# avabag01-ai/spectrogram-midi

Hardware: AMD Instinct MI355X
Metric: audio-seconds transcribed/sec (44.1 kHz, n_fft=2048) (higher is better)
Workload: dtype f64

## Files before the change

spectrogram-midi_amd/csrc/frame.hip:

```cpp
#include "kernels.h"
#include "fft8.h"
#include "frame_walk.h"
#include "pass_geometry.h"
#include "wave_ops.h"

#include <algorithm>
#include <cfloat>
#include <cmath>
#include <cstdlib>
#include <cstring>

namespace aegis {

constexpr int kFramesPerWg = 16;

constexpr size_t kFrameLdsFixed = (size_t)2048 * 16 + 2048 * 4 + 1040 * 4 + 128 * 4 + 16 * 4 + 256 * 4;

#if defined(AEGIS_ABLATE) && (AEGIS_ABLATE & 128)
__device__ long long g_frm_dbg[24];
#define FRM_TICK(k) { __builtin_amdgcn_s_waitcnt(0); const long long now__ = clock64(); facc[k] += now__ - flast; flast = now__; }
#else
#define FRM_TICK(k)
#endif
template <bool INJECT>
__global__ __launch_bounds__(256, 2) void frame_yin_kernel(PassParams p, DevTables tb, int frames_per_wg, int en_stride,
                                                           const double *__restrict__ inj) {
#if defined(AEGIS_ABLATE) && (AEGIS_ABLATE & 128)
    long long facc[12] = {0, 0, 0, 0, 0, 0, 0, 0, 0, 0, 0, 0}, flast = clock64();
#endif
    extern __shared__ __align__(16) unsigned char fsm[];
    double2 *z = reinterpret_cast<double2 *>(fsm);
    float *xs = reinterpret_cast<float *>(z + 2048);
    float *pw = xs + 2048;
    float *red = pw + 1040;
    float *blk = red + 128;
    float *part = blk + 16;
    float *en = part + 256;
    int64_t *frow = reinterpret_cast<int64_t *>(en + (size_t)frames_per_wg * en_stride);

    const int tid = threadIdx.x, lane = tid & 63, wid = tid >> 6;
    const int64_t n_sel = geo_n_sel(p);
    const int64_t fs0 = (int64_t)blockIdx.x * frames_per_wg;
    if (fs0 >= n_sel) return;
    const int nfr = (int)min((int64_t)frames_per_wg, n_sel - fs0);
    const bool want_pyin = (p.stages & 0x4u) != 0, want_mel = (p.stages & 0x3u) != 0;
    const bool want_rms = (p.stages & 0x8u) && p.out_rms != nullptr;
    const bool want_fft = (p.stages & 0x7u) != 0;
    const int mp = p.max_period;

    struct Geo { bool live; int c; int64_t base, n, start, f, o; };
    auto locate = [&](int i) {
        Geo g{false, 0, 0, 0, 0, 0, 0};
        g.live = i < nfr;
        if (g.live) {
            int64_t t;
            map_frame(p, fs0 + i, g.c, t, g.f);
            g.o = out_index(p, g.c, t);
            g.base = p.sample_off[g.c];
            g.n = p.sample_len[g.c];
            g.start = t * p.hop - 1024;
        }
        return g;
    };
    auto fetch = [&](const Geo &g, float (&v)[8]) {
#pragma unroll
        for (int r = 0; r < 8; ++r) {
            const int64_t idx = g.start + tid + r * 256;
            v[r] = (g.live && idx >= 0 && idx < g.n) ? p.pcm[g.base + idx] : 0.0f;
        }
    };
    auto locate_next = [&](const Geo &g, int i, int64_t sel_end) {
        if (i < nfr && g.live && fs0 + i < sel_end) {
            Geo n = g;
            n.start += p.hop; n.f += 1; n.o += 1;
            return n;
        }
        return locate(i);
    };
    Geo geo = locate(0);
    int64_t geo_sel_end = geo.live ? p.sel_off[geo.c + 1] : 0;
    float nx[8];
    fetch(geo, nx);
    Fft8Tw twr;

    const bool has_chunk = want_mel && tid < tb.mel_chunks;
    const int mel_bin = has_chunk ? tb.mel_chunk_bin[tid] : 0;
    int band_c0 = 0, band_c1 = 0;
    if (want_mel && (tid & 127) < p.n_mels) { band_c0 = tb.mel_band_chunk[tid & 127]; band_c1 = tb.mel_band_chunk[(tid & 127) + 1]; }
    float *pw1 = xs;
    float *part1 = xs + 1040;
    if (tid < 15) pw[1025 + tid] = 0.0f;

    if (want_pyin) {
        const Geo g0 = geo;
        Geo gl = g0;
        if (fs0 + nfr - 1 < geo_sel_end) { gl.start += (int64_t)(nfr - 1) * p.hop; } else gl = locate(nfr - 1);
        const int64_t span = (int64_t)(nfr - 1) * p.hop + 2048;
        const bool staged = g0.c == gl.c && p.hop == 512 && span + 4 * (span >> 9) <= 10240;
        float *stage = reinterpret_cast<float *>(z);
        if (staged) {
            const float *__restrict__ x0 = p.pcm + g0.base;
            const int n4 = (int)(span >> 2);
            float4 sv[10];
#pragma unroll
            for (int u = 0; u < 10; ++u) {
                const int q = tid + 256 * u;
                const int64_t idx = g0.start + 4 * (int64_t)q;
                float4 v = make_float4(0.0f, 0.0f, 0.0f, 0.0f);
                if (q < n4) {
                    if (idx >= 0 && idx + 3 < g0.n) {
                        typedef float f4u __attribute__((ext_vector_type(4), aligned(4)));
                        const f4u t = *reinterpret_cast<const f4u *>(x0 + idx);
                        v = make_float4(t.x, t.y, t.z, t.w);
                    } else {
                        if (idx >= 0 && idx < g0.n) v.x = x0[idx];
                        if (idx + 1 >= 0 && idx + 1 < g0.n) v.y = x0[idx + 1];
                        if (idx + 2 >= 0 && idx + 2 < g0.n) v.z = x0[idx + 2];
                        if (idx + 3 >= 0 && idx + 3 < g0.n) v.w = x0[idx + 3];
                    }
                }
                sv[u] = v;
            }
#pragma unroll
            for (int u = 0; u < 10; ++u) {
                const int q = tid + 256 * u;
                if (q < n4) {
                    const int i = 4 * q;
                    *reinterpret_cast<float4 *>(stage + i + 4 * (i >> 9)) =
                        make_float4(sv[u].x * sv[u].x, sv[u].y * sv[u].y, sv[u].z * sv[u].z, sv[u].w * sv[u].w);
                }
            }
            __syncthreads();
        }
        if (wid == 0) __builtin_amdgcn_s_setprio(3);
        if (wid == 0 && lane < nfr) {
            float *row = en + lane * en_stride;
            if (staged) {
                const float *srow = stage + lane * (512 + 4);
                energy_walk<true>([&](int j, float4 &a, float4 &b) {
                    const float *q = srow + j + 4 * (j >> 9);
                    a = *reinterpret_cast<const float4 *>(q);
                    b = *reinterpret_cast<const float4 *>(q + 4);
                }, row, mp);
            } else {
                const Geo g = locate(lane);
                const float *__restrict__ x = p.pcm + g.base;
                energy_walk_plain([&](int j) {
                    const int64_t q = g.start + j;
                    return (q >= 0 && q < g.n) ? x[q] : 0.0f;
                }, row, mp);
            }
        }
        if (wid == 0) __builtin_amdgcn_s_setprio(0);
        if (staged) __syncthreads();
    }
    if (want_fft) fft8_load_twiddles(twr, tb.twiddle, tid);
    FRM_TICK(0)
    __builtin_amdgcn_s_waitcnt(kWaitVmcnt0);

    for (int pr = 0; pr < nfr; pr += 2) {
        double2 P[2][4], Pn[2];
        int64_t fidx[2] = {0, 0};
        int64_t fout[2] = {0, 0};
        bool flive[2] = {false, false};
        int fclip[2] = {0, 0};
#pragma unroll
        for (int h = 0; h < 2; ++h) {
#pragma unroll
            for (int r = 0; r < 4; ++r) P[h][r] = make_double2(0.0, 0.0);
            Pn[h] = make_double2(0.0, 0.0);
            if (pr + h >= nfr) continue;
            const bool live = geo.live;
            const int c = geo.c;
            const int64_t f = geo.f, fo = geo.o;
            fidx[h] = f; flive[h] = live; fclip[h] = c;
            if constexpr (INJECT) fout[h] = fo;
            if (tid == 0) frow[pr + h] = live ? f : -1;
#pragma unroll
            for (int r = 0; r < 8; ++r) xs[tid + r * 256] = nx[r];
            {
                const int cprev = geo.c;
                geo = locate_next(geo, pr + h + 1, geo_sel_end);
                if (geo.live && geo.c != cprev) geo_sel_end = p.sel_off[geo.c + 1];
            }
            fetch(geo, nx);
            __syncthreads();
            FRM_TICK(1)

            if (want_rms && tid < 128) {
                const int bb = tid >> 3, a = tid & 7;
                const float *xb = xs + bb * 128 + a;
                float r = xb[0] * xb[0];
#pragma unroll
                for (int i = 1; i < 16; ++i) { const float v = xb[8 * i]; r = r + v * v; }
                red[tid] = r;
            }
            if (!want_fft) {
                __syncthreads();
                if (want_rms && tid < 16) {
                    const float *r = red + tid * 8;
                    blk[tid] = ((r[0] + r[1]) + (r[2] + r[3])) + ((r[4] + r[5]) + (r[6] + r[7]));
                }
                __syncthreads();
            } else {
                double2 v[8];
#pragma unroll
                for (int q = 0; q < 8; ++q) {
                    const int i = tid + 256 * q;
                    v[q] = make_double2((double)xs[i], i < 1024 ? (double)xs[1024 - i] : 0.0);
                }
                fft8_pass1_write(z, tid, v);
                __syncthreads();
                if (want_rms && tid < 16) {
                    const float *r = red + tid * 8;
                    blk[tid] = ((r[0] + r[1]) + (r[2] + r[3])) + ((r[4] + r[5]) + (r[6] + r[7]));
                }
                fft8_read8(z, tid, v);
                __syncthreads();
                fft8_pass_write<8>(z, tid, v, twr.p2);
                __syncthreads();
                fft8_read8(z, tid, v);
                __syncthreads();
                fft8_pass_write<64>(z, tid, v, twr.p3);
                __syncthreads();
                fft8_pass4(z, tid, twr);
                __syncthreads();
            }
            FRM_TICK(2)
            if (want_rms && tid == 0 && live) {
                float b0 = (blk[0] + blk[1]) + (blk[2] + blk[3]);
                float b1 = (blk[4] + blk[5]) + (blk[6] + blk[7]);
                float b2 = (blk[8] + blk[9]) + (blk[10] + blk[11]);
                float b3 = (blk[12] + blk[13]) + (blk[14] + blk[15]);
                const float total = 0.0f + ((b0 + b1) + (b2 + b3));
                p.out_rms[fo] = sqrtf(total / 2048.0f);
            }
            if (!want_fft) continue;

            {
                auto zpair = [&](int k, double2 &zk, double2 &zn) { zk = z[zsw(k & 2047)]; zn = z[zsw((2048 - k) & 2047)]; };
                auto Afrom = [](const double2 &zk, const double2 &zn) { return make_double2(zk.x + zn.x, zk.y - zn.y); };
                auto bin = [&](int k, const double2 &Am, const double2 &A, const double2 &Ap, const double2 &zk, const double2 &zn,
                               double2 &Pk) {
                    if (want_pyin) {
                        const double2 Bv = make_double2(zk.y + zn.y, zn.x - zk.x);
                        Pk = c_mul(A, Bv);
                    }
                    if (want_mel) {
                        const float re = (float)(0.125 * (2.0 * A.x - (Am.x + Ap.x)));
                        const float im = (float)(0.125 * (2.0 * A.y - (Am.y + Ap.y)));
                        const float mag = (float)sqrt((double)re * (double)re + (double)im * (double)im);
                        (h == 0 ? pw : pw1)[k] = mag * mag;
                    }
                };
                const int k0 = 4 * tid;
                double2 zk, zn, zk1, zn1;
                zpair(k0 - 1, zk, zn);
                double2 Am = Afrom(zk, zn);
                zpair(k0, zk, zn);
                double2 A = Afrom(zk, zn);
#pragma unroll
                for (int r = 0; r < 4; ++r) {
                    zpair(k0 + r + 1, zk1, zn1);
                    const double2 Ap = Afrom(zk1, zn1);
                    bin(k0 + r, Am, A, Ap, zk, zn, P[h][r]);
                    Am = A; A = Ap; zk = zk1; zn = zn1;
                }
                if (tid == 255) bin(1024, Am, A, make_double2(Am.x, -Am.y), zk, zn, Pn[h]);
            }
            if (want_mel && h == 1 && tid < 15) pw1[1025 + tid] = 0.0f;
            __syncthreads();
            FRM_TICK(3)
        }
        __builtin_amdgcn_s_waitcnt(kWaitVmcnt0);
        if (want_mel) {
            if (has_chunk) {
                const float4 *wp = reinterpret_cast<const float4 *>(tb.mel_chunk_w) + tid * 4;
                const float4 w0 = wp[0], w1 = wp[1], w2 = wp[2], w3 = wp[3];
#pragma unroll
                for (int h = 0; h < 2; ++h) {
                    const float *pp = (h == 0 ? pw : pw1) + mel_bin;
                    float acc = 0.0f;
                    acc = fmaf(w0.x, pp[0], acc); acc = fmaf(w0.y, pp[1], acc); acc = fmaf(w0.z, pp[2], acc); acc = fmaf(w0.w, pp[3], acc);
                    acc = fmaf(w1.x, pp[4], acc); acc = fmaf(w1.y, pp[5], acc); acc = fmaf(w1.z, pp[6], acc); acc = fmaf(w1.w, pp[7], acc);
                    acc = fmaf(w2.x, pp[8], acc); acc = fmaf(w2.y, pp[9], acc); acc = fmaf(w2.z, pp[10], acc); acc = fmaf(w2.w, pp[11], acc);
                    acc = fmaf(w3.x, pp[12], acc); acc = fmaf(w3.y, pp[13], acc); acc = fmaf(w3.z, pp[14], acc); acc = fmaf(w3.w, pp[15], acc);
                    (h == 0 ? part : part1)[tid] = acc;
                }
            }
            __syncthreads();
            {
                const int h = wid >> 1, bt = tid & 127;
                const bool live = flive[h];
                const float *pt = h == 0 ? part : part1;
                float acc = 0.0f;
                if (bt < p.n_mels && live) {
                    const int c0 = band_c0, c1 = band_c1;
                    float pv[6];
#pragma unroll
                    for (int k = 0; k < 6; ++k) pv[k] = pt[min(c0 + k, 255)];
                    acc = c0 < c1 ? pv[0] : 0.0f;
#pragma unroll
                    for (int k = 1; k < 6; ++k) if (c0 + k < c1) acc = acc + pv[k];
                    for (int cidx = c0 + 6; cidx < c1; ++cidx) acc = acc + pt[cidx];
                    p.melpow[fidx[h] * p.n_mels + bt] = acc;
                }
                const unsigned m = wave_umax(__float_as_uint(acc));
                if (lane == 0 && live) atomicMax(&p.clipmax[fclip[h]], m);
            }
            if (!want_pyin) __syncthreads();
        }
        FRM_TICK(4)
        if (!want_pyin) continue;

        {
#pragma unroll
            for (int r = 0; r < 4; ++r) {
                const int k = 4 * tid + r;
                const double2 u = P[0][r], v = P[1][r];
                z[zsw(k)] = make_double2(u.x - v.y, -u.y - v.x);
                if (k > 0) z[zsw(2048 - k)] = make_double2(u.x + v.y, u.y - v.x);
            }
            if (tid == 255) z[zsw(1024)] = make_double2(Pn[0].x - Pn[1].y, -Pn[0].y - Pn[1].x);
        }
        __syncthreads();
        {
            double2 v[8];
            fft8_read8(z, tid, v);
            __syncthreads();
            fft8_pass1_write(z, tid, v);
            __syncthreads();
            fft8_read8(z, tid, v);
            __syncthreads();
            fft8_pass_write<8>(z, tid, v, twr.p2);
            __syncthreads();
            fft8_read8(z, tid, v);
            __syncthreads();
            fft8_pass_write<64>(z, tid, v, twr.p3);
            __syncthreads();
            fft8_pass4_lags(z, tid, twr, mp);
            __syncthreads();
        }
        FRM_TICK(5)
        const bool keep_first = p.cmnd_in_frame != 0;
        if (keep_first) {
            float es[2][3];
#pragma unroll
            for (int h = 0; h < 2; ++h) {
                const float *row = en + (pr + h) * en_stride;
                float en0 = row[0];
                if (fabsf(en0) < 1e-6f) en0 = 0.0f;
#pragma unroll
                for (int u = 0; u < 3; ++u) {
                    float e = row[min(tid + 256 * u, mp)];
                    if (fabsf(e) < 1e-6f) e = 0.0f;
                    es[h][u] = en0 + e;
                }
            }
            __syncthreads();
            double *__restrict__ d0 = reinterpret_cast<double *>(en + pr * en_stride);
            double *__restrict__ d1 = p.dfn + fidx[1] * (int64_t)p.lag_stride;
#pragma unroll
            for (int u = 0; u < 3; ++u) {
                const int tau = tid + 256 * u;
                if (tau <= mp) {
                    const double2 zz = z[zsw(1024 + tau)];
                    double a0 = zz.x * (1.0 / 8192.0), a1 = -zz.y * (1.0 / 8192.0);
                    if (fabs(a0) < 1e-6) a0 = 0.0;
                    if (fabs(a1) < 1e-6) a1 = 0.0;
                    if constexpr (INJECT) {
                        if (flive[0]) d0[tau] = inj[fout[0] * (int64_t)(mp + 1) + tau];
                        if (flive[1]) d1[tau] = inj[fout[1] * (int64_t)(mp + 1) + tau];
                    } else {
                        if (flive[0]) d0[tau] = (double)es[0][u] - 2.0 * a0;
                        if (flive[1]) d1[tau] = (double)es[1][u] - 2.0 * a1;
                    }
                }
            }
        } else {
#pragma unroll
        for (int h = 0; h < 2; ++h) {
            if (!flive[h]) continue;
            const float *row = en + (pr + h) * en_stride;
            float en0 = row[0];
            if (fabsf(en0) < 1e-6f) en0 = 0.0f;
            double *__restrict__ drow = p.dfn + fidx[h] * (int64_t)p.lag_stride;
            for (int tau = tid; tau <= mp; tau += 256) {
                const double2 zz = z[zsw(1024 + tau)];
                double a = (h == 0 ? zz.x : -zz.y) * (1.0 / 8192.0);
                if (fabs(a) < 1e-6) a = 0.0;
                float e = row[tau];
                if (fabsf(e) < 1e-6f) e = 0.0f;
                const float esum = en0 + e;
                if constexpr (INJECT) drow[tau] = inj[fout[h] * (int64_t)(mp + 1) + tau];
                else drow[tau] = (double)esum - 2.0 * a;
            }
        }
        }
        FRM_TICK(6)
    }
    if (want_pyin && p.cmnd_in_frame) {
        const int RS = frame_cmnd_stride(mp), minp = p.min_period;
        double *zrows = reinterpret_cast<double *>(fsm);
        auto row_of = [&](int i) { return (i & 1) ? zrows + (i >> 1) * RS : reinterpret_cast<double *>(en + i * en_stride); };
        __syncthreads();
        double dv[kFramesPerWg][3];
        int64_t fr[kFramesPerWg];
#pragma unroll
        for (int i = 0; i < kFramesPerWg; ++i) fr[i] = i < nfr ? frow[i] : -1;
#pragma unroll
        for (int i = 0; i < kFramesPerWg; ++i) {
            const double *__restrict__ src = (i & 1) ? p.dfn + (fr[i] < 0 ? 0 : fr[i]) * (int64_t)p.lag_stride : row_of(i);
#pragma unroll
            for (int u = 0; u < 3; ++u) {
                const int tau = tid + 256 * u;
                dv[i][u] = (fr[i] >= 0 && tau <= mp) ? src[tau] : 0.0;
            }
        }
#pragma unroll
        for (int i = 1; i < kFramesPerWg; i += 2) {
#pragma unroll
            for (int u = 0; u < 3; ++u) {
                const int tau = tid + 256 * u;
                if (i < nfr && tau <= mp) zrows[(i >> 1) * RS + tau] = dv[i][u];
            }
        }
        __syncthreads();
        FRM_TICK(7)
        if (wid == 0) __builtin_amdgcn_s_setprio(3);
        if (wid == 0 && lane < nfr) cmnd_walk(row_of(lane), mp);
        if (wid == 0) __builtin_amdgcn_s_setprio(0);
        __syncthreads();
        FRM_TICK(8)
        const bool troughs = p.troughs != 0;
#pragma unroll
        for (int i = 0; i < kFramesPerWg; ++i) {
            double *__restrict__ drow = p.dfn + (fr[i] < 0 ? 0 : fr[i]) * (int64_t)p.lag_stride;
            double *__restrict__ cs = row_of(i);
#pragma unroll
            for (int u = 0; u < 3; ++u) {
                const int tau = tid + 256 * u;
                if (fr[i] >= 0 && tau >= minp && tau <= mp) {
                    const double yv = dv[i][u] / (cs[tau] / (double)tau + DBL_MIN);
                    if (troughs) cs[tau] = yv;
                    else drow[tau] = yv;
                }
            }
        }
        FRM_TICK(9)
        if (troughs) {
            __syncthreads();
            const int nl = p.n_lags, KM = trough_km(nl), NR = (nl + 63) >> 6;
            const unsigned long long below = (1ull << lane) - 1ull;
            for (int i = wid; i < nfr; i += 4) {
                if (fr[i] < 0) continue;
                const double *__restrict__ y = row_of(i) + minp;
                double *__restrict__ trow = p.dfn + fr[i] * (int64_t)p.lag_stride;
                int16_t *__restrict__ tiv = reinterpret_cast<int16_t *>(trow + 8 + 2 * KM);
                int K = 0;
                for (int r = 0; r < NR; ++r) {
                    const int k = 64 * r + lane;
                    bool tr = false;
                    double ym = 0.0, y0 = 0.0, yp = 0.0;
                    if (k < nl) {
                        y0 = y[k];
                        if (k > 0) ym = y[k - 1];
                        if (k < nl - 1) yp = y[k + 1];
                        if (k == 0) tr = y0 < yp;
                        else if (k == nl - 1) tr = y0 < ym;
                        else tr = (y0 < ym) && (y0 <= yp);
                    }
                    const unsigned long long m = __ballot(tr);
                    if (tr) {
                        const int pos = K + __popcll(m & below);
                        double shift = 0.0;
                        if (k > 0 && k < nl - 1) {
                            const double a = yp + ym - 2.0 * y0;
                            const double b = (yp - ym) / 2.0;
                            if (fabs(b) < fabs(a)) shift = -b / a;
                        }
                        trow[8 + pos] = y0;
                        trow[8 + KM + pos] = shift;
                        tiv[pos] = (int16_t)k;
                    }
                    K += __popcll(m);
                }
                if (lane == 0) trow[0] = __longlong_as_double((long long)K);
            }
        }
    }
#if defined(AEGIS_ABLATE) && (AEGIS_ABLATE & 128)
    if (blockIdx.x == 1000 && (tid == 0 || tid == 64)) { for (int k = 0; k < 10; ++k) g_frm_dbg[(tid ? 12 : 0) + k] = facc[k]; }
#endif
}
#if defined(AEGIS_ABLATE) && (AEGIS_ABLATE & 128)
hipError_t frame_debug_fetch(long long *dst) { return hipMemcpyFromSymbol(dst, HIP_SYMBOL(g_frm_dbg), sizeof(long long) * 24); }
#else
hipError_t frame_debug_fetch(long long *dst) { for (int i = 0; i < 24; ++i) dst[i] = 0; return hipSuccess; }
#endif
hipError_t frame_set_lds_limits() {
    hipError_t e = hipFuncSetAttribute(reinterpret_cast<const void *>(frame_yin_kernel<false>),
                                       hipFuncAttributeMaxDynamicSharedMemorySize, 160 * 1024);
    if (e != hipSuccess) return e;
    return hipFuncSetAttribute(reinterpret_cast<const void *>(frame_yin_kernel<true>),
                               hipFuncAttributeMaxDynamicSharedMemorySize, 160 * 1024);
}

int frame_batch_fpw(int max_period) {
    const int stride = frame_en_stride(max_period);
    int fpw = kFramesPerWg;
    while (fpw > 2 && kFrameLdsFixed + (size_t)fpw * stride * 4 > 80 * 1024) fpw -= 2;
    return fpw;
}
int trough_row_doubles_host(int n_lags) { return trough_row_doubles(n_lags); }
bool frame_cmnd_supported(int max_period) {
    if (max_period + 1 > 3 * 256) return false;
    const int stride = frame_en_stride(max_period), rs = frame_cmnd_stride(max_period);
    if (stride < max_period + 1) return false;
    for (int fpw : {2, frame_batch_fpw(max_period)})
        if ((size_t)(fpw / 2) * rs * 8 + 64 > kFrameLdsFixed) return false;
    return true;
}
void launch_frame(const PassParams &p, const DevTables &t, hipStream_t s, const double *inject_d) {
    if (p.n_sel == 0 || !(p.stages & 0xFu)) return;
    const int stride = frame_en_stride(p.max_period);
    const int fpw = p.n_sel >= 4096 ? frame_batch_fpw(p.max_period) : 2;
    size_t lds = kFrameLdsFixed + (size_t)fpw * stride * 4 + (size_t)fpw * 8;
    static const size_t lds_min = [] { const char *e = std::getenv("AEGIS_FRAME_LDS_MIN"); return e ? (size_t)std::atol(e) : (size_t)0; }();
    lds = std::max(lds, std::min<size_t>(lds_min, 160 * 1024));
    const dim3 grid((unsigned)((p.n_sel + fpw - 1) / fpw));
    if (inject_d) hipLaunchKernelGGL(frame_yin_kernel<true>, grid, dim3(256), lds, s, p, t, fpw, stride, inject_d);
    else hipLaunchKernelGGL(frame_yin_kernel<false>, grid, dim3(256), lds, s, p, t, fpw, stride, static_cast<const double *>(nullptr));
}

}
```

Measured before the change: 324,500.

## Batch LDS loads ahead of compute and hoist pyin spectrum write before mel

Groups LDS reads into register arrays ahead of sched_barriers in the RMS, FFT input and CMND normalisation loops so the loads are issued together rather than interleaved with arithmetic. Moves the mel weight global load and the pYIN power-spectrum write to z ahead of the vmcnt wait and mel reduction, and drops the separate barrier when mel runs. This is meant to hide LDS and global latency and remove a synchronisation point. In exchange it raises register pressure, adds unconditional loads of pw/pw1, and relies on z not being touched in the mel phase.

```diff
diff --git a/spectrogram-midi_amd/csrc/frame.hip b/spectrogram-midi_amd/csrc/frame.hip
--- a/spectrogram-midi_amd/csrc/frame.hip
+++ b/spectrogram-midi_amd/csrc/frame.hip
@@ -190,9 +190,13 @@
             if (want_rms && tid < 128) {
                 const int bb = tid >> 3, a = tid & 7;
                 const float *xb = xs + bb * 128 + a;
-                float r = xb[0] * xb[0];
-#pragma unroll
-                for (int i = 1; i < 16; ++i) { const float v = xb[8 * i]; r = r + v * v; }
+                float xv[16];
+#pragma unroll
+                for (int i = 0; i < 16; ++i) xv[i] = xb[8 * i];
+                __builtin_amdgcn_sched_barrier(0);
+                float r = xv[0] * xv[0];
+#pragma unroll
+                for (int i = 1; i < 16; ++i) r = r + xv[i] * xv[i];
                 red[tid] = r;
             }
             if (!want_fft) {
@@ -204,10 +208,15 @@
                 __syncthreads();
             } else {
                 double2 v[8];
-#pragma unroll
-                for (int q = 0; q < 8; ++q) {
-                    const int i = tid + 256 * q;
-                    v[q] = make_double2((double)xs[i], i < 1024 ? (double)xs[1024 - i] : 0.0);
+                {
+                    float xf[8], xr[4];
+#pragma unroll
+                    for (int q = 0; q < 8; ++q) xf[q] = xs[tid + 256 * q];
+#pragma unroll
+                    for (int q = 0; q < 4; ++q) xr[q] = xs[1024 - (tid + 256 * q)];
+                    __builtin_amdgcn_sched_barrier(0);
+#pragma unroll
+                    for (int q = 0; q < 8; ++q) v[q] = make_double2((double)xf[q], q < 4 ? (double)xr[q] : 0.0);
                 }
                 fft8_pass1_write(z, tid, v);
                 __syncthreads();
@@ -272,22 +281,36 @@
             __syncthreads();
             FRM_TICK(3)
         }
+        float4 w0 = make_float4(0.0f, 0.0f, 0.0f, 0.0f), w1 = w0, w2 = w0, w3 = w0;
+        if (has_chunk) {
+            const float4 *wp = reinterpret_cast<const float4 *>(tb.mel_chunk_w) + tid * 4;
+            w0 = wp[0]; w1 = wp[1]; w2 = wp[2]; w3 = wp[3];
+        }
+        if (__builtin_expect(want_pyin, 1)) {
+#pragma unroll
+            for (int r = 0; r < 4; ++r) {
+                const int k = 4 * tid + r;
+                const double2 u = P[0][r], v = P[1][r];
+                z[zsw(k)] = make_double2(u.x - v.y, -u.y - v.x);
+                if (k > 0) z[zsw(2048 - k)] = make_double2(u.x + v.y, u.y - v.x);
+            }
+            if (tid == 255) z[zsw(1024)] = make_double2(Pn[0].x - Pn[1].y, -Pn[0].y - Pn[1].x);
+        }
+        float pa[16], pb[16];
+#pragma unroll
+        for (int k = 0; k < 16; ++k) pa[k] = pw[mel_bin + k];
+#pragma unroll
+        for (int k = 0; k < 16; ++k) pb[k] = pw1[mel_bin + k];
+        __builtin_amdgcn_sched_barrier(0);
         __builtin_amdgcn_s_waitcnt(kWaitVmcnt0);
-        if (want_mel) {
-            if (has_chunk) {
-                const float4 *wp = reinterpret_cast<const float4 *>(tb.mel_chunk_w) + tid * 4;
-                const float4 w0 = wp[0], w1 = wp[1], w2 = wp[2], w3 = wp[3];
-#pragma unroll
-                for (int h = 0; h < 2; ++h) {
-                    const float *pp = (h == 0 ? pw : pw1) + mel_bin;
-                    float acc = 0.0f;
-                    acc = fmaf(w0.x, pp[0], acc); acc = fmaf(w0.y, pp[1], acc); acc = fmaf(w0.z, pp[2], acc); acc = fmaf(w0.w, pp[3], acc);
-                    acc = fmaf(w1.x, pp[4], acc); acc = fmaf(w1.y, pp[5], acc); acc = fmaf(w1.z, pp[6], acc); acc = fmaf(w1.w, pp[7], acc);
-                    acc = fmaf(w2.x, pp[8], acc); acc = fmaf(w2.y, pp[9], acc); acc = fmaf(w2.z, pp[10], acc); acc = fmaf(w2.w, pp[11], acc);
-                    acc = fmaf(w3.x, pp[12], acc); acc = fmaf(w3.y, pp[13], acc); acc = fmaf(w3.z, pp[14], acc); acc = fmaf(w3.w, pp[15], acc);
-                    (h == 0 ? part : part1)[tid] = acc;
-                }
-            }
+        if (__builtin_expect(want_mel, 1)) {
+            const float wv[16] = {w0.x, w0.y, w0.z, w0.w, w1.x, w1.y, w1.z, w1.w, w2.x, w2.y, w2.z, w2.w, w3.x, w3.y, w3.z, w3.w};
+            float acc0 = 0.0f, acc1 = 0.0f;
+#pragma unroll
+            for (int k = 0; k < 16; ++k) acc0 = fmaf(wv[k], pa[k], acc0);
+#pragma unroll
+            for (int k = 0; k < 16; ++k) acc1 = fmaf(wv[k], pb[k], acc1);
+            if (has_chunk) { part[tid] = acc0; part1[tid] = acc1; }
             __syncthreads();
             {
                 const int h = wid >> 1, bt = tid & 127;
@@ -313,17 +336,7 @@
         FRM_TICK(4)
         if (!want_pyin) continue;
 
-        {
-#pragma unroll
-            for (int r = 0; r < 4; ++r) {
-                const int k = 4 * tid + r;
-                const double2 u = P[0][r], v = P[1][r];
-                z[zsw(k)] = make_double2(u.x - v.y, -u.y - v.x);
-                if (k > 0) z[zsw(2048 - k)] = make_double2(u.x + v.y, u.y - v.x);
-            }
-            if (tid == 255) z[zsw(1024)] = make_double2(Pn[0].x - Pn[1].y, -Pn[0].y - Pn[1].x);
-        }
-        __syncthreads();
+        if (!want_mel) __syncthreads();
         {
             double2 v[8];
             fft8_read8(z, tid, v);
@@ -433,15 +446,25 @@
         __syncthreads();
         FRM_TICK(8)
         const bool troughs = p.troughs != 0;
+        auto q_live = [&](int i, int u) { const int tau = tid + 256 * u; return fr[i] >= 0 && tau >= minp && tau <= mp; };
+        auto cs_read = [&](int i, double (&c)[3]) {
+            const double *src = (i & 1) ? zrows + min(i >> 1, frames_per_wg / 2 - 1) * RS
+                                        : reinterpret_cast<const double *>(en + min(i, frames_per_wg - 2) * en_stride);
+#pragma unroll
+            for (int u = 0; u < 3; ++u) c[u] = src[min(tid + 256 * u, mp)];
+        };
 #pragma unroll
         for (int i = 0; i < kFramesPerWg; ++i) {
             double *__restrict__ drow = p.dfn + (fr[i] < 0 ? 0 : fr[i]) * (int64_t)p.lag_stride;
-            double *__restrict__ cs = row_of(i);
+            double *cs = row_of(i);
+            double cv[3];
+            cs_read(i, cv);
+            __builtin_amdgcn_sched_barrier(0);
 #pragma unroll
             for (int u = 0; u < 3; ++u) {
                 const int tau = tid + 256 * u;
-                if (fr[i] >= 0 && tau >= minp && tau <= mp) {
-                    const double yv = dv[i][u] / (cs[tau] / (double)tau + DBL_MIN);
+                if (q_live(i, u)) {
+                    const double yv = dv[i][u] / (cv[u] / (double)tau + DBL_MIN);
                     if (troughs) cs[tau] = yv;
                     else drow[tau] = yv;
                 }
```

Measured after the change: 333,300 (median of 6 runs). +2.7%, better.
